# hmmlillian/Neural-Color-Transfer

Hardware: AMD Instinct MI355X
Metric: 700x700 pairs/sec end-to-end L=5->1; PatchMatch HBM GB/s vs peak (higher is better)
Workload: dtype f32

## Files before the change

neural-color-transfer_amd/csrc/k_s1.hip:

```cpp
#include "nct_internal.h"
#include "nct_device.h"
#include "nct_reduce.h"
#include <cstdlib>
#include <rocprim/device/device_radix_sort.hpp>
#include <rocprim/device/device_scan.hpp>

#define LAB_D(u) ((double)(u) * (1.0 / 255.0))
#define LCHK() NCT_LAUNCH_CHECK()

constexpr int S1_SEG = NCT_S1_SEG;

struct S1Sys {
    int n, h, w;
    const double *daa, *dab, *dbb;
    const double *gx, *gy;
    const int* knn_id;
    nct_s1_graph g;
    int xcd;
    int one_xcd;
};
__device__ __forceinline__ int s1_one_xcd(int bid, int sel) { return (bid & 7) == sel - 1 ? (bid >> 3) : -1; }
__device__ __forceinline__ int s1_block_of(int bid, int nblocks, int xcd) {
    if (!xcd) return bid;
    const int q = nblocks >> 3, r = nblocks & 7, x = bid & 7, idx = bid >> 3;
    return (x < r ? x * (q + 1) : r * (q + 1) + (x - r) * q) + idx;
}
struct S1State { double gm[3], al[3], be[3]; int active[3], iters[3]; };

__device__ __forceinline__ void ld6(const double* __restrict__ v, size_t px, double (&o)[6]) {
    const double2* q = reinterpret_cast<const double2*>(v + px * 6);
    const double2 t0 = q[0], t1 = q[1], t2 = q[2];
    o[0] = t0.x; o[1] = t0.y; o[2] = t1.x; o[3] = t1.y; o[4] = t2.x; o[5] = t2.y;
}
__device__ __forceinline__ void st6(double* __restrict__ v, size_t px, const double (&o)[6]) {
    double2* q = reinterpret_cast<double2*>(v + px * 6);
    q[0] = make_double2(o[0], o[1]); q[1] = make_double2(o[2], o[3]); q[2] = make_double2(o[4], o[5]);
}
__device__ __forceinline__ int lo32(unsigned long long v) { return (int)(unsigned)(v & 0xFFFFFFFFull); }
__device__ __forceinline__ int hi32(unsigned long long v) { return (int)(unsigned)(v >> 32); }

__global__ void k_s1_iw2(const double* __restrict__ knn_w, int m, double nonlocalWeight, double* __restrict__ iw2) {
    const int e = blockIdx.x * blockDim.x + threadIdx.x;
    if (e >= m) return;
    const double iw = sqrt(knn_w[e]) * nonlocalWeight;
    iw2[e] = iw * iw;
}
__global__ void k_edge_keys(const int* __restrict__ knn_id, int m, unsigned* __restrict__ keys, unsigned* __restrict__ vals) {
    const int e = blockIdx.x * blockDim.x + threadIdx.x;
    if (e >= m) return;
    keys[e] = (unsigned)knn_id[e]; vals[e] = (unsigned)e;
}
__global__ void k_seg_starts(const unsigned* __restrict__ keys, int m, int* __restrict__ start, int n) {
    const int s = blockIdx.x * blockDim.x + threadIdx.x;
    if (s > n) return;
    int lo = 0, hi = m;
    while (lo < hi) { const int mid = (lo + hi) >> 1; if (keys[mid] < (unsigned)s) lo = mid + 1; else hi = mid; }
    start[s] = lo;
}
__global__ void k_s1_counts(const int* __restrict__ rev_start, int n, unsigned long long* __restrict__ cnt) {
    const int i = blockIdx.x * blockDim.x + threadIdx.x;
    if (i > n) return;
    unsigned long long v = 0;
    if (i < n) {
        const int deg = rev_start[i + 1] - rev_start[i];
        v = (unsigned long long)(deg < S1_SEG ? deg : S1_SEG) | ((unsigned long long)(deg > S1_SEG ? (deg - 1) / S1_SEG : 0) << 32);
    }
    cnt[i] = v;
}
__global__ void k_s1_sup_counts(const unsigned long long* __restrict__ starts, int n, int* __restrict__ cnt) {
    const int i = blockIdx.x * blockDim.x + threadIdx.x;
    if (i > n) return;
    int c = 0;
    if (i < n) { const int m = hi32(starts[i + 1]) - hi32(starts[i]); c = m > S1_SEG ? (m + S1_SEG - 1) / S1_SEG : 0; }
    cnt[i] = c;
}
__global__ void k_s1_sup_fill(const unsigned long long* __restrict__ starts, const int* __restrict__ sup_start, int n, int* __restrict__ sup_b0) {
    const int i = blockIdx.x * blockDim.x + threadIdx.x;
    if (i >= n) return;
    const int s0 = sup_start[i], ns = sup_start[i + 1] - s0, b0 = hi32(starts[i]);
    for (int k = 0; k < ns; ++k) sup_b0[s0 + k] = b0 + k * S1_SEG;
}
__global__ void k_s1_rev_build(const unsigned* __restrict__ keys_sorted, const unsigned* __restrict__ edge_sorted, const double* __restrict__ iw2, int m,
                               const int* __restrict__ rev_start, const unsigned long long* __restrict__ starts,
                               int* __restrict__ c_src, double* __restrict__ c_w, int* __restrict__ rev_src, double* __restrict__ rev_w,
                               int* __restrict__ seg_tgt, int* __restrict__ seg_e0) {
    const int e = blockIdx.x * blockDim.x + threadIdx.x;
    if (e >= m) return;
    const int t = (int)keys_sorted[e];
    const int rank = e - rev_start[t];
    const unsigned ed = edge_sorted[e];
    const int src = (int)(ed >> 3); const double wt = iw2[ed];
    const unsigned long long st = starts[t];
    if (rank < S1_SEG) { const int pos = lo32(st) + rank; c_src[pos] = src; c_w[pos] = wt; }
    else {
        rev_src[e] = src; rev_w[e] = wt;
        if ((rank & (S1_SEG - 1)) == 0) { const int sg = hi32(st) + rank / S1_SEG - 1; seg_tgt[sg] = t; seg_e0[sg] = e; }
    }
}

int nctk_s1_graph_build(nct_ctx* ctx, hipStream_t s, const int* knn_id, const double* knn_w, double nonlocalWeight, const nct_s1_graph& g, int* nseg_pinned) {
    const int n = g.n, m = 8 * n;
    DevBuf<unsigned> ek(ctx, m), ev(ctx, m), eks(ctx, m), evs(ctx, m);
    DevBuf<unsigned long long> cnt(ctx, (size_t)n + 1);
    DevBuf<int> scnt(ctx, (size_t)n + 1);
    if (!ek.ok() || !ev.ok() || !eks.ok() || !evs.ok() || !cnt.ok() || !scnt.ok()) return NCT_ERR_HIP;
    hipLaunchKernelGGL(k_s1_iw2, dim3(cdiv(m, 256)), dim3(256), 0, s, knn_w, m, nonlocalWeight, g.iw2); LCHK();
    hipLaunchKernelGGL(k_edge_keys, dim3(cdiv(m, 256)), dim3(256), 0, s, knn_id, m, (unsigned*)ek, (unsigned*)ev); LCHK();
    int end_bit = 1; while ((1u << end_bit) < (unsigned)n && end_bit < 32) ++end_bit;
    size_t tmp_bytes = 0, scan_bytes = 0, scan2_bytes = 0;
    NCT_HIP(rocprim::radix_sort_pairs(nullptr, tmp_bytes, (const unsigned*)ek, (unsigned*)eks, (const unsigned*)ev, (unsigned*)evs, m, 0, end_bit, s));
    NCT_HIP(rocprim::exclusive_scan(nullptr, scan_bytes, (const unsigned long long*)cnt, g.starts, 0ull, (size_t)n + 1, rocprim::plus<unsigned long long>(), s));
    NCT_HIP(rocprim::exclusive_scan(nullptr, scan2_bytes, (const int*)scnt, g.sup_start, 0, (size_t)n + 1, rocprim::plus<int>(), s));
    if (scan2_bytes > scan_bytes) scan_bytes = scan2_bytes;
    DevBuf<char> tmp(ctx, (tmp_bytes > scan_bytes ? tmp_bytes : scan_bytes) + 16);
    if (!tmp.ok()) return NCT_ERR_HIP;
    NCT_HIP(rocprim::radix_sort_pairs((void*)(char*)tmp, tmp_bytes, (const unsigned*)ek, (unsigned*)eks, (const unsigned*)ev, (unsigned*)evs, m, 0, end_bit, s));
    hipLaunchKernelGGL(k_seg_starts, dim3(cdiv(n + 1, 256)), dim3(256), 0, s, (const unsigned*)eks, m, g.rev_start, n); LCHK();
    hipLaunchKernelGGL(k_s1_counts, dim3(cdiv(n + 1, 256)), dim3(256), 0, s, (const int*)g.rev_start, n, (unsigned long long*)cnt); LCHK();
    NCT_HIP(rocprim::exclusive_scan((void*)(char*)tmp, scan_bytes, (const unsigned long long*)cnt, g.starts, 0ull, (size_t)n + 1, rocprim::plus<unsigned long long>(), s));
    hipLaunchKernelGGL(k_s1_rev_build, dim3(cdiv(m, 256)), dim3(256), 0, s, (const unsigned*)eks, (const unsigned*)evs, (const double*)g.iw2, m, (const int*)g.rev_start,
                       (const unsigned long long*)g.starts, g.c_src, g.c_w, g.rev_src, g.rev_w, g.seg_tgt, g.seg_e0); LCHK();
    hipLaunchKernelGGL(k_s1_sup_counts, dim3(cdiv(n + 1, 256)), dim3(256), 0, s, (const unsigned long long*)g.starts, n, (int*)scnt); LCHK();
    NCT_HIP(rocprim::exclusive_scan((void*)(char*)tmp, scan2_bytes, (const int*)scnt, g.sup_start, 0, (size_t)n + 1, rocprim::plus<int>(), s));
    hipLaunchKernelGGL(k_s1_sup_fill, dim3(cdiv(n, 256)), dim3(256), 0, s, (const unsigned long long*)g.starts, (const int*)g.sup_start, n, g.sup_b0); LCHK();
    if (nseg_pinned) {
        NCT_HIP(hipMemcpyAsync(nseg_pinned, (const char*)(g.starts + n) + 4, sizeof(int), hipMemcpyDeviceToHost, s));
        NCT_HIP(hipMemcpyAsync(nseg_pinned + 1, g.sup_start + n, sizeof(int), hipMemcpyDeviceToHost, s));
    }
    return 0;
}

__global__ void k_s1_setup(int n, const double* __restrict__ weight, float dWeight, const uint8_t* __restrict__ src, const uint8_t* __restrict__ ref,
                           double* __restrict__ daa, double* __restrict__ dab, double* __restrict__ dbb, double* __restrict__ rhs ) {
    const int i = blockIdx.x * blockDim.x + threadIdx.x;
    if (i >= n) return;
    const double dw = sqrt(weight[i]) * (double)sqrtf(dWeight);
#pragma unroll
    for (int c = 0; c < 3; ++c) {
        const double v0 = dw * LAB_D(src[(size_t)i * 3 + c]);
        const double rb = dw * LAB_D(ref[(size_t)i * 3 + c]);
        daa[(size_t)i * 3 + c] = v0 * v0; dab[(size_t)i * 3 + c] = v0 * dw; dbb[(size_t)i * 3 + c] = dw * dw;
        rhs[(size_t)i * 3 + c] = v0 * rb; rhs[(size_t)(n + i) * 3 + c] = dw * rb;
    }
}

__global__ __launch_bounds__(256) void k_s1_hub(nct_s1_graph G, const double* __restrict__ v ) {
    const int nseg = hi32(G.starts[G.n]);
    const int lane = threadIdx.x & 63;
    for (int sg = blockIdx.x * 4 + (threadIdx.x >> 6); sg < nseg; sg += gridDim.x * 4) {
        const int t = G.seg_tgt[sg];
        const int e = G.seg_e0[sg] + lane;
        const bool in = e < G.rev_start[t + 1];
        double term[6], vt[6], vj[6];
        int j = t; double wt = 0.0;
        if (in) { j = G.rev_src[e]; wt = G.rev_w[e]; }
        ld6(v, (size_t)t, vt); ld6(v, (size_t)j, vj);
#pragma unroll
        for (int c = 0; c < 6; ++c) { const double d = wt * (vt[c] - vj[c]); term[c] = in ? d : 0.0; }
#pragma unroll
        for (int off = 32; off >= 1; off >>= 1)
#pragma unroll
            for (int c = 0; c < 6; ++c) term[c] += __shfl_xor(term[c], off);
        if (lane == 0) {
#pragma unroll
            for (int c = 0; c < 6; ++c) G.hub_part[(size_t)sg * 6 + c] = term[c];
        }
    }
}

__global__ __launch_bounds__(256) void k_s1_hub2(nct_s1_graph G) {
    const int nsup = G.sup_start[G.n];
    const int lane = threadIdx.x & 63;
    for (int sb = blockIdx.x * 4 + (threadIdx.x >> 6); sb < nsup; sb += gridDim.x * 4) {
        const int b0 = G.sup_b0[sb];
        const int t = G.seg_tgt[b0];
        const int bend = min(b0 + S1_SEG, hi32(G.starts[t + 1]));
        double term[6];
        const bool in = b0 + lane < bend;
        if (in) ld6(G.hub_part, (size_t)(b0 + lane), term);
#pragma unroll
        for (int c = 0; c < 6; ++c) term[c] = in ? term[c] : 0.0;
#pragma unroll
        for (int off = 32; off >= 1; off >>= 1)
#pragma unroll
            for (int c = 0; c < 6; ++c) term[c] += __shfl_xor(term[c], off);
        if (lane == 0) st6(G.sup_part, (size_t)sb, term);
    }
}

#ifndef NCT_S1_CHUNK
#define NCT_S1_CHUNK 1024
#endif
constexpr int S1_CHUNK = NCT_S1_CHUNK;
template <bool COOP>
__device__ __forceinline__ void s1_op(const S1Sys& S, const double* __restrict__ p, int i, bool live, double (&a)[3], double (&b)[3], double (&ya)[3], double (&yb)[3], int lb = -1) {
    const int w = S.w, h = S.h;
    int e0 = 0, e1 = 0, h0 = 0, h1 = 0;
#pragma unroll
    for (int c = 0; c < 3; ++c) { a[c] = 0.0; b[c] = 0.0; ya[c] = 0.0; yb[c] = 0.0; }
    if (live) {
        const int y = i / w, x = i - y * w;
        { double own[6]; ld6(p, (size_t)i, own);
#pragma unroll
          for (int c = 0; c < 3; ++c) { a[c] = own[c]; b[c] = own[3 + c]; } }
#pragma unroll
        for (int c = 0; c < 3; ++c) {
            ya[c] = S.daa[(size_t)i * 3 + c] * a[c] + S.dab[(size_t)i * 3 + c] * b[c];
            yb[c] = S.dab[(size_t)i * 3 + c] * a[c] + S.dbb[(size_t)i * 3 + c] * b[c];
        }
        auto edge = [&](int j, double wt) {
            double q[6]; ld6(p, (size_t)j, q);
#pragma unroll
            for (int c = 0; c < 3; ++c) { ya[c] += wt * (a[c] - q[c]); yb[c] += wt * (b[c] - q[3 + c]); }
        };
        {
            const bool ex[4] = {x + 1 < w, x > 0, y + 1 < h, y > 0};
            const int nj[4] = {ex[0] ? i + 1 : i, ex[1] ? i - 1 : i, ex[2] ? i + w : i, ex[3] ? i - w : i};
            const double g4[4] = {S.gx[i], S.gx[ex[1] ? i - 1 : i], S.gy[i], S.gy[ex[3] ? i - w : i]};
            double q4[4][6];
#pragma unroll
            for (int u = 0; u < 4; ++u) ld6(p, (size_t)nj[u], q4[u]);
#pragma unroll
            for (int u = 0; u < 4; ++u)
                if (ex[u]) {
                    const double wt = 2.0 * (g4[u] * g4[u]);
#pragma unroll
                    for (int c = 0; c < 3; ++c) { ya[c] += wt * (a[c] - q4[u][c]); yb[c] += wt * (b[c] - q4[u][3 + c]); }
                }
        }
#pragma unroll
        for (int k = 0; k < 8; ++k) edge(S.knn_id[(size_t)i * 8 + k], S.g.iw2[(size_t)i * 8 + k]);
        const unsigned long long s0 = S.g.starts[i], s1 = S.g.starts[i + 1];
        e0 = lo32(s0); e1 = lo32(s1); h0 = hi32(s0); h1 = hi32(s1);
    }
    if constexpr (!COOP) {
        if (live) {
            int e = e0;
            for (; e + 4 <= e1; e += 4) {
                int j[4]; double wt[4], pv[4][6];
#pragma unroll
                for (int u = 0; u < 4; ++u) { j[u] = S.g.c_src[e + u]; wt[u] = S.g.c_w[e + u]; }
#pragma unroll
                for (int u = 0; u < 4; ++u) ld6(p, (size_t)j[u], pv[u]);
#pragma unroll
                for (int u = 0; u < 4; ++u)
#pragma unroll
                    for (int c = 0; c < 3; ++c) { ya[c] += wt[u] * (a[c] - pv[u][c]); yb[c] += wt[u] * (b[c] - pv[u][3 + c]); }
            }
            for (; e < e1; ++e) {
                const int j = S.g.c_src[e]; const double wt = S.g.c_w[e];
                double q[6]; ld6(p, (size_t)j, q);
#pragma unroll
                for (int c = 0; c < 3; ++c) { ya[c] += wt * (a[c] - q[c]); yb[c] += wt * (b[c] - q[3 + c]); }
            }
        }
    } else {
        __shared__ double s_pv[6 * S1_CHUNK];
        __shared__ double s_wt[S1_CHUNK];
        const int i0 = (lb >= 0 ? lb : (int)blockIdx.x) * 256, i1 = min(i0 + 256, S.n);
        const int E0 = lo32(S.g.starts[i0]), E1 = lo32(S.g.starts[i1]);
        for (int base = E0; base < E1; base += S1_CHUNK) {
            const int cnt = min(S1_CHUNK, E1 - base);
            for (int t = threadIdx.x; t < cnt; t += 256) {
                const int j = S.g.c_src[base + t];
                s_wt[t] = S.g.c_w[base + t];
                double q[6]; ld6(p, (size_t)j, q);
#pragma unroll
                for (int c = 0; c < 6; ++c) s_pv[c * S1_CHUNK + t] = q[c];
            }
            __syncthreads();
            const int lo = max(e0, base) - base, hi = min(e1, base + cnt) - base;
            for (int t = lo; t < hi; ++t) {
                const double wt = s_wt[t];
#pragma unroll
                for (int c = 0; c < 3; ++c) { ya[c] += wt * (a[c] - s_pv[c * S1_CHUNK + t]); yb[c] += wt * (b[c] - s_pv[(3 + c) * S1_CHUNK + t]); }
            }
            __syncthreads();
        }
    }
    bool sup = false;
    if (h1 - h0 > S1_SEG) { h0 = S.g.sup_start[i]; h1 = S.g.sup_start[i + 1]; sup = true; }
    const double* __restrict__ part = sup ? S.g.sup_part : S.g.hub_part;
    for (int sg = h0; sg < h1; ++sg) {
        double q[6]; ld6(part, (size_t)sg, q);
#pragma unroll
        for (int c = 0; c < 3; ++c) { ya[c] += q[c]; yb[c] += q[3 + c]; }
    }
}

template <bool COOP>
__global__ __launch_bounds__(256) void k_s1_residual(S1Sys S, const double* __restrict__ x6, const double* __restrict__ rhs, double* __restrict__ r6) {
    const int i = blockIdx.x * 256 + threadIdx.x;
    double a[3], b[3], ya[3], yb[3];
    s1_op<COOP>(S, x6, i, i < S.n, a, b, ya, yb);
    if (i < S.n) {
        double o[6];
#pragma unroll
        for (int c = 0; c < 3; ++c) { o[c] = rhs[(size_t)i * 3 + c] - ya[c]; o[3 + c] = rhs[(size_t)(S.n + i) * 3 + c] - yb[c]; }
        st6(r6, (size_t)i, o);
    }
}
template <bool COOP>
__global__ __launch_bounds__(256) void k_s1_apply(S1Sys S, const double* __restrict__ r6, double* __restrict__ w6, double* __restrict__ partial ) {
    const int lb = S.one_xcd ? s1_one_xcd(blockIdx.x, S.one_xcd) : s1_block_of(blockIdx.x, gridDim.x, S.xcd);
    if (lb < 0) return;
    const int i = lb * 256 + threadIdx.x;
    double acc[6] = {0, 0, 0, 0, 0, 0};
    double a[3], b[3], ya[3], yb[3];
    s1_op<COOP>(S, r6, i, i < S.n, a, b, ya, yb, lb);
    if (i < S.n) {
#pragma unroll
        for (int c = 0; c < 3; ++c) {
            acc[c] = a[c] * a[c] + b[c] * b[c];
            acc[3 + c] = a[c] * ya[c] + b[c] * yb[c];
        }
        const double o[6] = {ya[0], ya[1], ya[2], yb[0], yb[1], yb[2]};
        st6(w6, (size_t)i, o);
    }
    block_reduce_store<6>(acc, partial, lb);
}

__device__ __forceinline__ void s1_scalars(bool first, const double (&sm)[6], const S1State* __restrict__ in, double tol2, S1State& o) {
#pragma unroll
    for (int c = 0; c < 3; ++c) {
        if (first) {
            const double g0 = sm[c]; const bool act = g0 > tol2;
            o.gm[c] = g0; o.be[c] = 0.0; o.al[c] = act ? g0 / sm[3 + c] : 0.0; o.active[c] = act ? 1 : 0; o.iters[c] = act ? 1 : 0;
        } else if (in->active[c]) {
            const double g1 = sm[c];
            const double be = g1 / in->gm[c];
            const double al = g1 / (sm[3 + c] - (be * g1) / in->al[c]);
            const bool act = g1 > tol2;
            o.gm[c] = g1; o.be[c] = be; o.al[c] = al; o.active[c] = act ? 1 : 0; o.iters[c] = in->iters[c] + (act ? 1 : 0);
        } else {
            o.gm[c] = in->gm[c]; o.be[c] = in->be[c]; o.al[c] = in->al[c]; o.active[c] = 0; o.iters[c] = in->iters[c];
        }
    }
}
__global__ __launch_bounds__(256) void k_s1_scal(const double* __restrict__ partial, int nb, const S1State* __restrict__ in, S1State* __restrict__ out, int first, double tol2) {
    double sm[6]; final_reduce<6>(partial, nb, sm);
    if (threadIdx.x == 0) { S1State o; s1_scalars(first != 0, sm, in, tol2, o); *out = o; }
}
constexpr int S1_FUSE_NB = 512;
template <bool FUSED>
__global__ __launch_bounds__(256) void k_s1_update(int n, int nb, const double* __restrict__ partial, const S1State* __restrict__ sin, S1State* __restrict__ sout,
                                                   int first_scal, double tol2, int first_vec, double* __restrict__ r6, const double* __restrict__ w6,
                                                   double* __restrict__ p6, double* __restrict__ s6, double* __restrict__ x6, int one_xcd) {
    const int bid = one_xcd ? s1_one_xcd(blockIdx.x, one_xcd) : (int)blockIdx.x;
    if (bid < 0) return;
    const size_t total = (size_t)3 * n;
    const size_t base = (size_t)bid * 768 + threadIdx.x;
    double2 rv[3], wv[3], pv[3], sv[3], xv[3];
    const double2* r2 = reinterpret_cast<const double2*>(r6); const double2* w2 = reinterpret_cast<const double2*>(w6);
    const double2* x2 = reinterpret_cast<const double2*>(x6); const double2* p2 = reinterpret_cast<const double2*>(p6); const double2* s2 = reinterpret_cast<const double2*>(s6);
#pragma unroll
    for (int k = 0; k < 3; ++k) {
        const size_t g0 = base + (size_t)k * 256, g = g0 < total ? g0 : total - 1;
        rv[k] = r2[g]; wv[k] = w2[g]; xv[k] = x2[g];
        pv[k] = p2[g]; sv[k] = s2[g];
        if (first_vec) { pv[k] = make_double2(0.0, 0.0); sv[k] = make_double2(0.0, 0.0); }
    }
    double al[3], be[3]; bool act[3];
    if constexpr (FUSED) {
        double sm[6]; final_reduce<6>(partial, nb, sm);
        S1State o; s1_scalars(first_scal != 0, sm, sin, tol2, o);
        if (bid == 0 && threadIdx.x == 0) *sout = o;
#pragma unroll
        for (int c = 0; c < 3; ++c) { al[c] = o.al[c]; be[c] = o.be[c]; act[c] = o.active[c] != 0; }
    } else {
#pragma unroll
        for (int c = 0; c < 3; ++c) { al[c] = sin->al[c]; be[c] = sin->be[c]; act[c] = sin->active[c] != 0; }
    }
    double2* r2o = reinterpret_cast<double2*>(r6); double2* x2o = reinterpret_cast<double2*>(x6); double2* p2o = reinterpret_cast<double2*>(p6); double2* s2o = reinterpret_cast<double2*>(s6);
#pragma unroll
    for (int k = 0; k < 3; ++k) {
        const size_t g = base + (size_t)k * 256;
        if (g >= total) continue;
        const int c0 = (int)((2 * g) % 3), c1 = (c0 + 1) % 3;
        const double a0 = c0 == 0 ? al[0] : (c0 == 1 ? al[1] : al[2]), b0 = c0 == 0 ? be[0] : (c0 == 1 ? be[1] : be[2]);
        const double a1 = c1 == 0 ? al[0] : (c1 == 1 ? al[1] : al[2]), b1 = c1 == 0 ? be[0] : (c1 == 1 ? be[1] : be[2]);
        const bool on0 = c0 == 0 ? act[0] : (c0 == 1 ? act[1] : act[2]), on1 = c1 == 0 ? act[0] : (c1 == 1 ? act[1] : act[2]);
        double2 pn, sn, xn, rn;
        pn.x = first_vec ? rv[k].x : b0 * pv[k].x + rv[k].x;  pn.y = first_vec ? rv[k].y : b1 * pv[k].y + rv[k].y;
        sn.x = first_vec ? wv[k].x : b0 * sv[k].x + wv[k].x;  sn.y = first_vec ? wv[k].y : b1 * sv[k].y + wv[k].y;
        xn.x = xv[k].x + a0 * pn.x;  xn.y = xv[k].y + a1 * pn.y;
        rn.x = rv[k].x - a0 * sn.x;  rn.y = rv[k].y - a1 * sn.y;
        if (!on0) { pn.x = pv[k].x; sn.x = sv[k].x; xn.x = xv[k].x; rn.x = rv[k].x; }
        if (!on1) { pn.y = pv[k].y; sn.y = sv[k].y; xn.y = xv[k].y; rn.y = rv[k].y; }
        if (on0 || on1) { p2o[g] = pn; s2o[g] = sn; x2o[g] = xn; r2o[g] = rn; }
    }
}
__global__ void k_pack6(int n, const double* __restrict__ x, double* __restrict__ x6) {
    const int i = blockIdx.x * blockDim.x + threadIdx.x;
    if (i >= 2 * n * 3) return;
    const int c = i % 3, part = i / (n * 3), px = (i - part * n * 3) / 3;
    x6[(size_t)px * 6 + part * 3 + c] = x[i];
}
__global__ void k_unpack6(int n, const double* __restrict__ x6, double* __restrict__ x) {
    const int i = blockIdx.x * blockDim.x + threadIdx.x;
    if (i >= 2 * n * 3) return;
    const int c = i % 3, part = i / (n * 3), px = (i - part * n * 3) / 3;
    x[i] = x6[(size_t)px * 6 + part * 3 + c];
}

int nctk_s1_solve(nct_ctx* ctx, hipStream_t s, const nct_s1_graph& g, const int* knn_id, const double* weight, float dWeight, const uint8_t* s_lab_level,
                  const uint8_t* g_lab_level, const double* gx, const double* gy, int layer, int h, int w, double* x, int* cg_iters_host ) {
    const int n = h * w, nbl = cdiv(n, 256);
    DevBuf<double> daa(ctx, (size_t)3 * n), dab(ctx, (size_t)3 * n), dbb(ctx, (size_t)3 * n), rhs(ctx, (size_t)6 * n);
    DevBuf<double> x6(ctx, (size_t)6 * n), r6(ctx, (size_t)6 * n), w6(ctx, (size_t)6 * n), p6(ctx, (size_t)6 * n), s6(ctx, (size_t)6 * n), partial(ctx, (size_t)nbl * 6);
    DevBuf<S1State> st(ctx, 2);
    if (!daa.ok() || !dab.ok() || !dbb.ok() || !rhs.ok() || !x6.ok() || !r6.ok() || !w6.ok() || !p6.ok() || !s6.ok() || !partial.ok() || !st.ok()) return NCT_ERR_HIP;
    hipLaunchKernelGGL(k_s1_setup, dim3(nbl), dim3(256), 0, s, n, weight, dWeight, s_lab_level, g_lab_level, (double*)daa, (double*)dab, (double*)dbb, (double*)rhs); LCHK();
    static const int s1_xcd = [] { const char* e = getenv("NCT_S1_XCD"); return e ? atoi(e) : 1; }();
    static const int s1_one_max = [] { const char* e = getenv("NCT_S1_ONE_XCD_MAX"); return e ? atoi(e) : 32; }();
    const int one_xcd = (nbl <= s1_one_max && nbl <= S1_FUSE_NB) ? 1 + (ctx->home_xcd & 7) : 0;
    const int ogrid = one_xcd ? nbl * 8 : nbl;
    S1Sys S{n, h, w, daa, dab, dbb, gx, gy, knn_id, g, (s1_xcd && n >= 100000) ? 1 : 0, one_xcd};
    const double tol2 = 1e-6 * 1e-6;
    const int maxit = layer == 4 ? 50 : 100;
    const bool coop = n >= 100000;
    const bool fused = nbl <= S1_FUSE_NB;
    const int hub_blind = cdiv(cdiv(8 * n, S1_SEG), 4) < 256 ? cdiv(cdiv(8 * n, S1_SEG), 4) : 256;
    const int hub_grid = g.nseg_hint == 0 ? 0 : (g.nseg_hint > 0 ? (cdiv(g.nseg_hint, 4) < 4096 ? cdiv(g.nseg_hint, 4) : 4096) : hub_blind);
    const int hub2_grid = (g.nseg_hint == 0 || g.nsup_hint == 0) ? 0 : (g.nsup_hint > 0 ? (cdiv(g.nsup_hint, 4) < 1024 ? cdiv(g.nsup_hint, 4) : 1024) : (cdiv(hub_blind, S1_SEG) < 64 ? cdiv(hub_blind, S1_SEG) : 64));
    auto hub = [&](const double* v) -> int {
        if (hub_grid) { hipLaunchKernelGGL(k_s1_hub, dim3(hub_grid), dim3(256), 0, s, g, v); LCHK(); }
        if (hub2_grid) { hipLaunchKernelGGL(k_s1_hub2, dim3(hub2_grid), dim3(256), 0, s, g); LCHK(); }
        return 0;
    };
    auto apply = [&](bool kt) -> int {
        if (kt) { int rk = ctx->kt_begin(s, NCT_KT_S1_APPLY); if (rk) return rk; }
        if (coop) hipLaunchKernelGGL(k_s1_apply<true>, dim3(nbl), dim3(256), 0, s, S, (const double*)r6, (double*)w6, (double*)partial);
        else      hipLaunchKernelGGL(k_s1_apply<false>, dim3(ogrid), dim3(256), 0, s, S, (const double*)r6, (double*)w6, (double*)partial);
        LCHK();
        if (kt) { int rk = ctx->kt_end(s); if (rk) return rk; }
        return 0;
    };
    hipLaunchKernelGGL(k_pack6, dim3(cdiv(6 * n, 256)), dim3(256), 0, s, n, (const double*)x, (double*)x6); LCHK();
    { int rc = hub(x6); if (rc) return rc; }
    if (coop) hipLaunchKernelGGL(k_s1_residual<true>, dim3(nbl), dim3(256), 0, s, S, (const double*)x6, (const double*)rhs, (double*)r6);
    else      hipLaunchKernelGGL(k_s1_residual<false>, dim3(nbl), dim3(256), 0, s, S, (const double*)x6, (const double*)rhs, (double*)r6);
    LCHK();
    { int rc = hub(r6); if (rc) return rc; rc = apply(false); if (rc) return rc; }
    S1State* slot[2] = {(S1State*)st, (S1State*)st + 1};
    for (int k = 1; k <= maxit; ++k) {
        const bool kt = ctx->kt_on && layer == 4 && k >= 3 && k < 11;
        if (fused) {
            hipLaunchKernelGGL(k_s1_update<true>, dim3(ogrid), dim3(256), 0, s, n, nbl, (const double*)partial, (const S1State*)slot[k & 1], slot[(k - 1) & 1], k == 1 ? 1 : 0, tol2,
                               k == 1 ? 1 : 0, (double*)r6, (const double*)w6, (double*)p6, (double*)s6, (double*)x6, one_xcd); LCHK();
        } else {
            if (kt) { int rk = ctx->kt_begin(s, NCT_KT_S1_SCALARS); if (rk) return rk; }
            hipLaunchKernelGGL(k_s1_scal, dim3(1), dim3(256), 0, s, (const double*)partial, nbl, (const S1State*)slot[k & 1], slot[(k - 1) & 1], k == 1 ? 1 : 0, tol2); LCHK();
            if (kt) { int rk = ctx->kt_end(s); if (rk) return rk; rk = ctx->kt_begin(s, NCT_KT_S1_UPDATE); if (rk) return rk; }
            hipLaunchKernelGGL(k_s1_update<false>, dim3(nbl), dim3(256), 0, s, n, nbl, (const double*)partial, (const S1State*)slot[(k - 1) & 1], slot[(k - 1) & 1], 0, tol2,
                               k == 1 ? 1 : 0, (double*)r6, (const double*)w6, (double*)p6, (double*)s6, (double*)x6, 0); LCHK();
            if (kt) { int rk = ctx->kt_end(s); if (rk) return rk; }
        }
        if (k < maxit) { int rc = hub(r6); if (rc) return rc; rc = apply(kt); if (rc) return rc; }
    }
    hipLaunchKernelGGL(k_unpack6, dim3(cdiv(6 * n, 256)), dim3(256), 0, s, n, (const double*)x6, x); LCHK();
    if (cg_iters_host) {
        S1State hst;
        NCT_HIP(hipMemcpyAsync(&hst, slot[(maxit - 1) & 1], sizeof hst, hipMemcpyDeviceToHost, s));
        NCT_HIP(hipStreamSynchronize(s));
        for (int c = 0; c < 3; ++c) cg_iters_host[c] = hst.iters[c];
    }
    return 0;
}
```

Baseline: 14.72.

## Recompute S1 diagonal coefficients on the fly and pad residual rows with packed constants

Drops the three per-pixel diagonal arrays (daa, dab, dbb) and recomputes them inside the operator from the pixel weight and the packed 8-bit source Lab values. On the large non-fused path these values live in the padding slot of an 8-double-stride residual row, so they arrive in the same cache lines as the residual. On the fused path they sit in a small separate double2 array. This cuts memory traffic in the CG apply and residual kernels, at the cost of a strided residual layout, extra index arithmetic in the update kernel, and more template variants.

```diff
diff --git a/neural-color-transfer_amd/csrc/k_s1.hip b/neural-color-transfer_amd/csrc/k_s1.hip
--- a/neural-color-transfer_amd/csrc/k_s1.hip
+++ b/neural-color-transfer_amd/csrc/k_s1.hip
@@ -12,7 +12,6 @@
 
 struct S1Sys {
     int n, h, w;
-    const double *daa, *dab, *dbb;
     const double *gx, *gy;
     const int* knn_id;
     nct_s1_graph g;
@@ -27,14 +26,21 @@
 }
 struct S1State { double gm[3], al[3], be[3]; int active[3], iters[3]; };
 
+constexpr int S1_RS = 8;
+template <int ST = 6>
 __device__ __forceinline__ void ld6(const double* __restrict__ v, size_t px, double (&o)[6]) {
-    const double2* q = reinterpret_cast<const double2*>(v + px * 6);
+    const double2* q = reinterpret_cast<const double2*>(v + px * ST);
     const double2 t0 = q[0], t1 = q[1], t2 = q[2];
     o[0] = t0.x; o[1] = t0.y; o[2] = t1.x; o[3] = t1.y; o[4] = t2.x; o[5] = t2.y;
 }
+template <int ST = 6>
 __device__ __forceinline__ void st6(double* __restrict__ v, size_t px, const double (&o)[6]) {
-    double2* q = reinterpret_cast<double2*>(v + px * 6);
+    double2* q = reinterpret_cast<double2*>(v + px * ST);
     q[0] = make_double2(o[0], o[1]); q[1] = make_double2(o[2], o[3]); q[2] = make_double2(o[4], o[5]);
+}
+__device__ __forceinline__ double2 s1_pad(double dw, const uint8_t* __restrict__ lab) {
+    const unsigned long long u = (unsigned long long)lab[0] | ((unsigned long long)lab[1] << 16) | ((unsigned long long)lab[2] << 32);
+    return make_double2(dw, __longlong_as_double((long long)u));
 }
 __device__ __forceinline__ int lo32(unsigned long long v) { return (int)(unsigned)(v & 0xFFFFFFFFull); }
 __device__ __forceinline__ int hi32(unsigned long long v) { return (int)(unsigned)(v >> 32); }
@@ -131,7 +137,7 @@
 }
 
 __global__ void k_s1_setup(int n, const double* __restrict__ weight, float dWeight, const uint8_t* __restrict__ src, const uint8_t* __restrict__ ref,
-                           double* __restrict__ daa, double* __restrict__ dab, double* __restrict__ dbb, double* __restrict__ rhs ) {
+                           double2* __restrict__ cst, int cs , double* __restrict__ rhs ) {
     const int i = blockIdx.x * blockDim.x + threadIdx.x;
     if (i >= n) return;
     const double dw = sqrt(weight[i]) * (double)sqrtf(dWeight);
@@ -139,11 +145,12 @@
     for (int c = 0; c < 3; ++c) {
         const double v0 = dw * LAB_D(src[(size_t)i * 3 + c]);
         const double rb = dw * LAB_D(ref[(size_t)i * 3 + c]);
-        daa[(size_t)i * 3 + c] = v0 * v0; dab[(size_t)i * 3 + c] = v0 * dw; dbb[(size_t)i * 3 + c] = dw * dw;
         rhs[(size_t)i * 3 + c] = v0 * rb; rhs[(size_t)(n + i) * 3 + c] = dw * rb;
     }
-}
-
+    cst[(size_t)i * cs] = s1_pad(dw, src + (size_t)i * 3);
+}
+
+template <int ST>
 __global__ __launch_bounds__(256) void k_s1_hub(nct_s1_graph G, const double* __restrict__ v ) {
     const int nseg = hi32(G.starts[G.n]);
     const int lane = threadIdx.x & 63;
@@ -154,7 +161,7 @@
         double term[6], vt[6], vj[6];
         int j = t; double wt = 0.0;
         if (in) { j = G.rev_src[e]; wt = G.rev_w[e]; }
-        ld6(v, (size_t)t, vt); ld6(v, (size_t)j, vj);
+        ld6<ST>(v, (size_t)t, vt); ld6<ST>(v, (size_t)j, vj);
 #pragma unroll
         for (int c = 0; c < 6; ++c) { const double d = wt * (vt[c] - vj[c]); term[c] = in ? d : 0.0; }
 #pragma unroll
@@ -192,24 +199,21 @@
 #define NCT_S1_CHUNK 1024
 #endif
 constexpr int S1_CHUNK = NCT_S1_CHUNK;
-template <bool COOP>
-__device__ __forceinline__ void s1_op(const S1Sys& S, const double* __restrict__ p, int i, bool live, double (&a)[3], double (&b)[3], double (&ya)[3], double (&yb)[3], int lb = -1) {
+template <bool COOP, int ST>
+__device__ __forceinline__ void s1_op(const S1Sys& S, const double* __restrict__ p, const double2* cst, int cs, int i, bool live, double (&a)[3], double (&b)[3], double (&ya)[3], double (&yb)[3],
+                                      int lb = -1) {
     const int w = S.w, h = S.h;
     int e0 = 0, e1 = 0, h0 = 0, h1 = 0;
 #pragma unroll
     for (int c = 0; c < 3; ++c) { a[c] = 0.0; b[c] = 0.0; ya[c] = 0.0; yb[c] = 0.0; }
     if (live) {
         const int y = i / w, x = i - y * w;
-        { double own[6]; ld6(p, (size_t)i, own);
-#pragma unroll
-          for (int c = 0; c < 3; ++c) { a[c] = own[c]; b[c] = own[3 + c]; } }
-#pragma unroll
-        for (int c = 0; c < 3; ++c) {
-            ya[c] = S.daa[(size_t)i * 3 + c] * a[c] + S.dab[(size_t)i * 3 + c] * b[c];
-            yb[c] = S.dab[(size_t)i * 3 + c] * a[c] + S.dbb[(size_t)i * 3 + c] * b[c];
-        }
+        double own[6]; ld6<ST>(p, (size_t)i, own);
+        const double2 pd = cst[(size_t)i * cs];
+#pragma unroll
+        for (int c = 0; c < 3; ++c) { a[c] = own[c]; b[c] = own[3 + c]; }
         auto edge = [&](int j, double wt) {
-            double q[6]; ld6(p, (size_t)j, q);
+            double q[6]; ld6<ST>(p, (size_t)j, q);
 #pragma unroll
             for (int c = 0; c < 3; ++c) { ya[c] += wt * (a[c] - q[c]); yb[c] += wt * (b[c] - q[3 + c]); }
         };
@@ -219,7 +223,16 @@
             const double g4[4] = {S.gx[i], S.gx[ex[1] ? i - 1 : i], S.gy[i], S.gy[ex[3] ? i - w : i]};
             double q4[4][6];
 #pragma unroll
-            for (int u = 0; u < 4; ++u) ld6(p, (size_t)nj[u], q4[u]);
+            for (int u = 0; u < 4; ++u) ld6<ST>(p, (size_t)nj[u], q4[u]);
+            __builtin_amdgcn_sched_barrier(0);
+            const double dw = pd.x; const unsigned long long lab = (unsigned long long)__double_as_longlong(pd.y);
+#pragma unroll
+            for (int c = 0; c < 3; ++c) {
+                const double v0 = dw * LAB_D((unsigned)((lab >> (16 * c)) & 0xFFu));
+                const double daa = v0 * v0, dab = v0 * dw, dbb = dw * dw;
+                ya[c] = daa * a[c] + dab * b[c];
+                yb[c] = dab * a[c] + dbb * b[c];
+            }
 #pragma unroll
             for (int u = 0; u < 4; ++u)
                 if (ex[u]) {
@@ -241,7 +254,7 @@
 #pragma unroll
                 for (int u = 0; u < 4; ++u) { j[u] = S.g.c_src[e + u]; wt[u] = S.g.c_w[e + u]; }
 #pragma unroll
-                for (int u = 0; u < 4; ++u) ld6(p, (size_t)j[u], pv[u]);
+                for (int u = 0; u < 4; ++u) ld6<ST>(p, (size_t)j[u], pv[u]);
 #pragma unroll
                 for (int u = 0; u < 4; ++u)
 #pragma unroll
@@ -249,7 +262,7 @@
             }
             for (; e < e1; ++e) {
                 const int j = S.g.c_src[e]; const double wt = S.g.c_w[e];
-                double q[6]; ld6(p, (size_t)j, q);
+                double q[6]; ld6<ST>(p, (size_t)j, q);
 #pragma unroll
                 for (int c = 0; c < 3; ++c) { ya[c] += wt * (a[c] - q[c]); yb[c] += wt * (b[c] - q[3 + c]); }
             }
@@ -264,7 +277,7 @@
             for (int t = threadIdx.x; t < cnt; t += 256) {
                 const int j = S.g.c_src[base + t];
                 s_wt[t] = S.g.c_w[base + t];
-                double q[6]; ld6(p, (size_t)j, q);
+                double q[6]; ld6<ST>(p, (size_t)j, q);
 #pragma unroll
                 for (int c = 0; c < 6; ++c) s_pv[c * S1_CHUNK + t] = q[c];
             }
@@ -288,26 +301,29 @@
     }
 }
 
-template <bool COOP>
-__global__ __launch_bounds__(256) void k_s1_residual(S1Sys S, const double* __restrict__ x6, const double* __restrict__ rhs, double* __restrict__ r6) {
+template <bool COOP, int RS>
+__global__ __launch_bounds__(256) void k_s1_residual(S1Sys S, const double* __restrict__ x6, const double2* __restrict__ cst, const double* __restrict__ rhs, double* __restrict__ r) {
     const int i = blockIdx.x * 256 + threadIdx.x;
     double a[3], b[3], ya[3], yb[3];
-    s1_op<COOP>(S, x6, i, i < S.n, a, b, ya, yb);
+    if constexpr (RS == S1_RS) s1_op<COOP, 6>(S, x6, reinterpret_cast<const double2*>(r) + 3, 4, i, i < S.n, a, b, ya, yb);
+    else                       s1_op<COOP, 6>(S, x6, cst, 1, i, i < S.n, a, b, ya, yb);
     if (i < S.n) {
         double o[6];
 #pragma unroll
         for (int c = 0; c < 3; ++c) { o[c] = rhs[(size_t)i * 3 + c] - ya[c]; o[3 + c] = rhs[(size_t)(S.n + i) * 3 + c] - yb[c]; }
-        st6(r6, (size_t)i, o);
-    }
-}
-template <bool COOP>
-__global__ __launch_bounds__(256) void k_s1_apply(S1Sys S, const double* __restrict__ r6, double* __restrict__ w6, double* __restrict__ partial ) {
+        st6<RS>(r, (size_t)i, o);
+    }
+}
+template <bool COOP, int RS>
+__device__ __forceinline__ void s1_apply(const S1Sys& S, const double* __restrict__ r , const double2* __restrict__ cst, double* __restrict__ w6,
+                                         double* __restrict__ partial ) {
     const int lb = S.one_xcd ? s1_one_xcd(blockIdx.x, S.one_xcd) : s1_block_of(blockIdx.x, gridDim.x, S.xcd);
     if (lb < 0) return;
     const int i = lb * 256 + threadIdx.x;
     double acc[6] = {0, 0, 0, 0, 0, 0};
     double a[3], b[3], ya[3], yb[3];
-    s1_op<COOP>(S, r6, i, i < S.n, a, b, ya, yb, lb);
+    if constexpr (RS == S1_RS) s1_op<COOP, RS>(S, r, reinterpret_cast<const double2*>(r) + 3, 4, i, i < S.n, a, b, ya, yb, lb);
+    else                       s1_op<COOP, RS>(S, r, cst, 1, i, i < S.n, a, b, ya, yb, lb);
     if (i < S.n) {
 #pragma unroll
         for (int c = 0; c < 3; ++c) {
@@ -318,6 +334,14 @@
         st6(w6, (size_t)i, o);
     }
     block_reduce_store<6>(acc, partial, lb);
+}
+template <bool COOP>
+__global__ __launch_bounds__(256) void k_s1_apply(S1Sys S, const double* __restrict__ r, const double2* __restrict__ cst, double* __restrict__ w6, double* __restrict__ partial) {
+    s1_apply<COOP, S1_RS>(S, r, cst, w6, partial);
+}
+template <bool COOP>
+__global__ __launch_bounds__(256) void k_s1_apply48(S1Sys S, const double* __restrict__ r, const double2* __restrict__ cst, double* __restrict__ w6, double* __restrict__ partial) {
+    s1_apply<COOP, 6>(S, r, cst, w6, partial);
 }
 
 __device__ __forceinline__ void s1_scalars(bool first, const double (&sm)[6], const S1State* __restrict__ in, double tol2, S1State& o) {
@@ -344,19 +368,20 @@
 constexpr int S1_FUSE_NB = 512;
 template <bool FUSED>
 __global__ __launch_bounds__(256) void k_s1_update(int n, int nb, const double* __restrict__ partial, const S1State* __restrict__ sin, S1State* __restrict__ sout,
-                                                   int first_scal, double tol2, int first_vec, double* __restrict__ r6, const double* __restrict__ w6,
+                                                   int first_scal, double tol2, int first_vec, double* __restrict__ r, const double* __restrict__ w6,
                                                    double* __restrict__ p6, double* __restrict__ s6, double* __restrict__ x6, int one_xcd) {
+    constexpr int RS = FUSED ? 6 : S1_RS;
     const int bid = one_xcd ? s1_one_xcd(blockIdx.x, one_xcd) : (int)blockIdx.x;
     if (bid < 0) return;
     const size_t total = (size_t)3 * n;
     const size_t base = (size_t)bid * 768 + threadIdx.x;
     double2 rv[3], wv[3], pv[3], sv[3], xv[3];
-    const double2* r2 = reinterpret_cast<const double2*>(r6); const double2* w2 = reinterpret_cast<const double2*>(w6);
+    const double2* r2 = reinterpret_cast<const double2*>(r); const double2* w2 = reinterpret_cast<const double2*>(w6);
     const double2* x2 = reinterpret_cast<const double2*>(x6); const double2* p2 = reinterpret_cast<const double2*>(p6); const double2* s2 = reinterpret_cast<const double2*>(s6);
 #pragma unroll
     for (int k = 0; k < 3; ++k) {
         const size_t g0 = base + (size_t)k * 256, g = g0 < total ? g0 : total - 1;
-        rv[k] = r2[g]; wv[k] = w2[g]; xv[k] = x2[g];
+        rv[k] = r2[RS == S1_RS ? g + (unsigned)g / 3u : g]; wv[k] = w2[g]; xv[k] = x2[g];
         pv[k] = p2[g]; sv[k] = s2[g];
         if (first_vec) { pv[k] = make_double2(0.0, 0.0); sv[k] = make_double2(0.0, 0.0); }
     }
@@ -371,7 +396,7 @@
 #pragma unroll
         for (int c = 0; c < 3; ++c) { al[c] = sin->al[c]; be[c] = sin->be[c]; act[c] = sin->active[c] != 0; }
     }
-    double2* r2o = reinterpret_cast<double2*>(r6); double2* x2o = reinterpret_cast<double2*>(x6); double2* p2o = reinterpret_cast<double2*>(p6); double2* s2o = reinterpret_cast<double2*>(s6);
+    double2* r2o = reinterpret_cast<double2*>(r); double2* x2o = reinterpret_cast<double2*>(x6); double2* p2o = reinterpret_cast<double2*>(p6); double2* s2o = reinterpret_cast<double2*>(s6);
 #pragma unroll
     for (int k = 0; k < 3; ++k) {
         const size_t g = base + (size_t)k * 256;
@@ -387,7 +412,7 @@
         rn.x = rv[k].x - a0 * sn.x;  rn.y = rv[k].y - a1 * sn.y;
         if (!on0) { pn.x = pv[k].x; sn.x = sv[k].x; xn.x = xv[k].x; rn.x = rv[k].x; }
         if (!on1) { pn.y = pv[k].y; sn.y = sv[k].y; xn.y = xv[k].y; rn.y = rv[k].y; }
-        if (on0 || on1) { p2o[g] = pn; s2o[g] = sn; x2o[g] = xn; r2o[g] = rn; }
+        if (on0 || on1) { p2o[g] = pn; s2o[g] = sn; x2o[g] = xn; r2o[RS == S1_RS ? g + (unsigned)g / 3u : g] = rn; }
     }
 }
 __global__ void k_pack6(int n, const double* __restrict__ x, double* __restrict__ x6) {
@@ -406,57 +431,66 @@
 int nctk_s1_solve(nct_ctx* ctx, hipStream_t s, const nct_s1_graph& g, const int* knn_id, const double* weight, float dWeight, const uint8_t* s_lab_level,
                   const uint8_t* g_lab_level, const double* gx, const double* gy, int layer, int h, int w, double* x, int* cg_iters_host ) {
     const int n = h * w, nbl = cdiv(n, 256);
-    DevBuf<double> daa(ctx, (size_t)3 * n), dab(ctx, (size_t)3 * n), dbb(ctx, (size_t)3 * n), rhs(ctx, (size_t)6 * n);
-    DevBuf<double> x6(ctx, (size_t)6 * n), r6(ctx, (size_t)6 * n), w6(ctx, (size_t)6 * n), p6(ctx, (size_t)6 * n), s6(ctx, (size_t)6 * n), partial(ctx, (size_t)nbl * 6);
+    const bool fused = nbl <= S1_FUSE_NB;
+    const int rs = fused ? 6 : S1_RS;
+    DevBuf<double> rhs(ctx, (size_t)6 * n);
+    DevBuf<double> x6(ctx, (size_t)6 * n), r(ctx, (size_t)rs * n), w6(ctx, (size_t)6 * n), p6(ctx, (size_t)6 * n), s6(ctx, (size_t)6 * n), partial(ctx, (size_t)nbl * 6);
+    DevBuf<double2> cst(ctx, fused ? (size_t)n : 1);
     DevBuf<S1State> st(ctx, 2);
-    if (!daa.ok() || !dab.ok() || !dbb.ok() || !rhs.ok() || !x6.ok() || !r6.ok() || !w6.ok() || !p6.ok() || !s6.ok() || !partial.ok() || !st.ok()) return NCT_ERR_HIP;
-    hipLaunchKernelGGL(k_s1_setup, dim3(nbl), dim3(256), 0, s, n, weight, dWeight, s_lab_level, g_lab_level, (double*)daa, (double*)dab, (double*)dbb, (double*)rhs); LCHK();
+    if (!rhs.ok() || !x6.ok() || !r.ok() || !cst.ok() || !w6.ok() || !p6.ok() || !s6.ok() || !partial.ok() || !st.ok()) return NCT_ERR_HIP;
+    hipLaunchKernelGGL(k_s1_setup, dim3(nbl), dim3(256), 0, s, n, weight, dWeight, s_lab_level, g_lab_level, fused ? (double2*)cst : (double2*)(double*)r + 3, fused ? 1 : 4,
+                       (double*)rhs); LCHK();
     static const int s1_xcd = [] { const char* e = getenv("NCT_S1_XCD"); return e ? atoi(e) : 1; }();
     static const int s1_one_max = [] { const char* e = getenv("NCT_S1_ONE_XCD_MAX"); return e ? atoi(e) : 32; }();
     const int one_xcd = (nbl <= s1_one_max && nbl <= S1_FUSE_NB) ? 1 + (ctx->home_xcd & 7) : 0;
     const int ogrid = one_xcd ? nbl * 8 : nbl;
-    S1Sys S{n, h, w, daa, dab, dbb, gx, gy, knn_id, g, (s1_xcd && n >= 100000) ? 1 : 0, one_xcd};
+    S1Sys S{n, h, w, gx, gy, knn_id, g, (s1_xcd && n >= 100000) ? 1 : 0, one_xcd};
     const double tol2 = 1e-6 * 1e-6;
     const int maxit = layer == 4 ? 50 : 100;
     const bool coop = n >= 100000;
-    const bool fused = nbl <= S1_FUSE_NB;
     const int hub_blind = cdiv(cdiv(8 * n, S1_SEG), 4) < 256 ? cdiv(cdiv(8 * n, S1_SEG), 4) : 256;
     const int hub_grid = g.nseg_hint == 0 ? 0 : (g.nseg_hint > 0 ? (cdiv(g.nseg_hint, 4) < 4096 ? cdiv(g.nseg_hint, 4) : 4096) : hub_blind);
     const int hub2_grid = (g.nseg_hint == 0 || g.nsup_hint == 0) ? 0 : (g.nsup_hint > 0 ? (cdiv(g.nsup_hint, 4) < 1024 ? cdiv(g.nsup_hint, 4) : 1024) : (cdiv(hub_blind, S1_SEG) < 64 ? cdiv(hub_blind, S1_SEG) : 64));
-    auto hub = [&](const double* v) -> int {
-        if (hub_grid) { hipLaunchKernelGGL(k_s1_hub, dim3(hub_grid), dim3(256), 0, s, g, v); LCHK(); }
+    auto hub = [&](const double* v, int vs) -> int {
+        if (hub_grid) {
+            if (vs == S1_RS) hipLaunchKernelGGL(k_s1_hub<S1_RS>, dim3(hub_grid), dim3(256), 0, s, g, v);
+            else   hipLaunchKernelGGL(k_s1_hub<6>, dim3(hub_grid), dim3(256), 0, s, g, v);
+            LCHK();
+        }
         if (hub2_grid) { hipLaunchKernelGGL(k_s1_hub2, dim3(hub2_grid), dim3(256), 0, s, g); LCHK(); }
         return 0;
     };
     auto apply = [&](bool kt) -> int {
         if (kt) { int rk = ctx->kt_begin(s, NCT_KT_S1_APPLY); if (rk) return rk; }
-        if (coop) hipLaunchKernelGGL(k_s1_apply<true>, dim3(nbl), dim3(256), 0, s, S, (const double*)r6, (double*)w6, (double*)partial);
-        else      hipLaunchKernelGGL(k_s1_apply<false>, dim3(ogrid), dim3(256), 0, s, S, (const double*)r6, (double*)w6, (double*)partial);
+        if (!fused)    hipLaunchKernelGGL(k_s1_apply<true>, dim3(nbl), dim3(256), 0, s, S, (const double*)r, (const double2*)cst, (double*)w6, (double*)partial);
+        else if (coop) hipLaunchKernelGGL(k_s1_apply48<true>, dim3(nbl), dim3(256), 0, s, S, (const double*)r, (const double2*)cst, (double*)w6, (double*)partial);
+        else           hipLaunchKernelGGL(k_s1_apply48<false>, dim3(ogrid), dim3(256), 0, s, S, (const double*)r, (const double2*)cst, (double*)w6, (double*)partial);
         LCHK();
         if (kt) { int rk = ctx->kt_end(s); if (rk) return rk; }
         return 0;
     };
     hipLaunchKernelGGL(k_pack6, dim3(cdiv(6 * n, 256)), dim3(256), 0, s, n, (const double*)x, (double*)x6); LCHK();
-    { int rc = hub(x6); if (rc) return rc; }
-    if (coop) hipLaunchKernelGGL(k_s1_residual<true>, dim3(nbl), dim3(256), 0, s, S, (const double*)x6, (const double*)rhs, (double*)r6);
-    else      hipLaunchKernelGGL(k_s1_residual<false>, dim3(nbl), dim3(256), 0, s, S, (const double*)x6, (const double*)rhs, (double*)r6);
+    { int rc = hub(x6, 6); if (rc) return rc; }
+    if (!fused)    hipLaunchKernelGGL(HIP_KERNEL_NAME(k_s1_residual<true, S1_RS>), dim3(nbl), dim3(256), 0, s, S, (const double*)x6, (const double2*)cst, (const double*)rhs, (double*)r);
+    else if (coop) hipLaunchKernelGGL(HIP_KERNEL_NAME(k_s1_residual<true, 6>), dim3(nbl), dim3(256), 0, s, S, (const double*)x6, (const double2*)cst, (const double*)rhs, (double*)r);
+    else           hipLaunchKernelGGL(HIP_KERNEL_NAME(k_s1_residual<false, 6>), dim3(nbl), dim3(256), 0, s, S, (const double*)x6, (const double2*)cst, (const double*)rhs, (double*)r);
     LCHK();
-    { int rc = hub(r6); if (rc) return rc; rc = apply(false); if (rc) return rc; }
+    { int rc = hub(r, rs); if (rc) return rc; rc = apply(false); if (rc) return rc; }
     S1State* slot[2] = {(S1State*)st, (S1State*)st + 1};
     for (int k = 1; k <= maxit; ++k) {
         const bool kt = ctx->kt_on && layer == 4 && k >= 3 && k < 11;
         if (fused) {
             hipLaunchKernelGGL(k_s1_update<true>, dim3(ogrid), dim3(256), 0, s, n, nbl, (const double*)partial, (const S1State*)slot[k & 1], slot[(k - 1) & 1], k == 1 ? 1 : 0, tol2,
-                               k == 1 ? 1 : 0, (double*)r6, (const double*)w6, (double*)p6, (double*)s6, (double*)x6, one_xcd); LCHK();
+                               k == 1 ? 1 : 0, (double*)r, (const double*)w6, (double*)p6, (double*)s6, (double*)x6, one_xcd); LCHK();
         } else {
             if (kt) { int rk = ctx->kt_begin(s, NCT_KT_S1_SCALARS); if (rk) return rk; }
             hipLaunchKernelGGL(k_s1_scal, dim3(1), dim3(256), 0, s, (const double*)partial, nbl, (const S1State*)slot[k & 1], slot[(k - 1) & 1], k == 1 ? 1 : 0, tol2); LCHK();
             if (kt) { int rk = ctx->kt_end(s); if (rk) return rk; rk = ctx->kt_begin(s, NCT_KT_S1_UPDATE); if (rk) return rk; }
             hipLaunchKernelGGL(k_s1_update<false>, dim3(nbl), dim3(256), 0, s, n, nbl, (const double*)partial, (const S1State*)slot[(k - 1) & 1], slot[(k - 1) & 1], 0, tol2,
-                               k == 1 ? 1 : 0, (double*)r6, (const double*)w6, (double*)p6, (double*)s6, (double*)x6, 0); LCHK();
+                               k == 1 ? 1 : 0, (double*)r, (const double*)w6, (double*)p6, (double*)s6, (double*)x6, 0); LCHK();
             if (kt) { int rk = ctx->kt_end(s); if (rk) return rk; }
         }
-        if (k < maxit) { int rc = hub(r6); if (rc) return rc; rc = apply(kt); if (rc) return rc; }
+        if (k < maxit) { int rc = hub(r, rs); if (rc) return rc; rc = apply(kt); if (rc) return rc; }
     }
     hipLaunchKernelGGL(k_unpack6, dim3(cdiv(6 * n, 256)), dim3(256), 0, s, n, (const double*)x6, x); LCHK();
     if (cg_iters_host) {
```

New measurement: 14.87, median of 6. 1.1% higher.
